# ZECTBynmo/iris-tts

Measured on AMD Instinct MI355X. Metric: audio samples/sec (22.05 kHz) on 80-mel x 1000-frame batch, higher is better.
Workload: dtype f32

## Files before the change

iris-tts_amd/csrc/mrf_pair_bf16.h:

```cpp
#pragma once
#include <stdio.h>
#include "conv_mfma_bf16.h"
#ifndef IRIS_B16_RES_EARLY
#define IRIS_B16_RES_EARLY 1
#endif

#ifndef IRIS_B16_RING_TAIL_GUARD
#define IRIS_B16_RING_TAIL_GUARD 1
#endif
#ifndef IRIS_B16_PAIR_SUM_DEFAULT
#define IRIS_B16_PAIR_SUM_DEFAULT 1
#endif
#ifndef IRIS_B16_SUM32_MT
#define IRIS_B16_SUM32_MT 3
#endif
#ifndef IRIS_B16_SUM64_MT
#define IRIS_B16_SUM64_MT 3
#endif
#ifndef IRIS_B16_SUM32_MINB
#define IRIS_B16_SUM32_MINB 2
#endif
#ifndef IRIS_B16_SUM64_MINB
#define IRIS_B16_SUM64_MINB 2
#endif

namespace iris {
namespace b16 {

struct PairProblem {
    const uint16_t* x;
    const void* w1;
    const void* w2;
    const float* b1;
    const float* b2;
    uint16_t* y;
    int ks;
    int dil;
};

struct PairLaunch {
    PairProblem p[kMaxGroup];
    int B, L, C;
    float slope;
    int nz;
    int Qp, n_ct;
    int n_jobs;
    int jobs_per_xcd;
    int bias_off;
    void* sum_y;
    int sum_f32;
    float inv_n;
};

constexpr int kPairSpanMax = 50;

__device__ __forceinline__ float lrelu_max(float v, float slope) { return fmaxf(v, v * slope); }

template <int NT, int CIC, int D>
__device__ __forceinline__ void ring_request(u32x4 (&wv)[D][NT], __amdgpu_buffer_rsrc_t wr, unsigned wvoff,
                                             unsigned q_bytes, unsigned tap_bytes) {
    constexpr int QPC = CIC / 16;
    constexpr int QL = QPC == 8 ? 3 : (QPC == 4 ? 2 : (QPC == 2 ? 1 : 0));
#pragma unroll
    for (int i = 0; i < D; ++i) {
#pragma unroll
        for (int nt = 0; nt < NT; ++nt)
            wv[i][nt] = buf_load4(wr, wvoff + (unsigned)nt * 1024u, (unsigned)(i >> QL) * tap_bytes + (unsigned)(i & (QPC - 1)) * q_bytes);
        __builtin_amdgcn_sched_barrier(0);
    }
}

template <int MT, int NT, int CIC, int D>
__device__ __forceinline__ void ring_mma_loop(f32x16 (&acc)[MT][NT], u32x4 (&wv)[D][NT], const char* a_lane, int dil_bytes,
                                              __amdgpu_buffer_rsrc_t wr, unsigned wvoff, unsigned q_bytes,
                                              unsigned tap_bytes, int ks) {
    constexpr int QPC = CIC / 16;
    constexpr int QL = QPC == 8 ? 3 : (QPC == 4 ? 2 : (QPC == 2 ? 1 : 0));
    constexpr int SB = CIC * 2 + 16;
    const int NG = ks * QPC;
    auto w_soff = [&](int n) -> unsigned { return (unsigned)(n >> QL) * tap_bytes + (unsigned)(n & (QPC - 1)) * q_bytes; };
    auto load_a = [&](u32x4 (&av)[MT], int n) {
        int tap = n >> QL;
        tap = tap < ks ? tap : ks - 1;
        const char* ap = a_lane + tap * dil_bytes + (n & (QPC - 1)) * 32;
#pragma unroll
        for (int m = 0; m < MT; ++m) av[m] = *reinterpret_cast<const u32x4*>(ap + m * 32 * SB);
    };
    u32x4 av[2][MT];
    load_a(av[0], 0);
    auto group = [&](int i, int n) {
        load_a(av[(i + 1) & 1], n + 1);
        __builtin_amdgcn_sched_barrier(0);
#pragma unroll
        for (int nt = 0; nt < NT; ++nt)
#pragma unroll
            for (int m = 0; m < MT; ++m)
                acc[m][nt] = __builtin_amdgcn_mfma_f32_32x32x16_bf16(
                    __builtin_bit_cast(bf16x8, wv[i][nt]), __builtin_bit_cast(bf16x8, av[i & 1][m]), acc[m][nt], 0, 0, 0);
        __builtin_amdgcn_sched_barrier(0);
#pragma unroll
        for (int nt = 0; nt < NT; ++nt)
            wv[i][nt] = buf_load4(wr, wvoff + (unsigned)nt * 1024u, w_soff(n + D));
    };
    constexpr bool kTail = IRIS_B16_RING_TAIL_GUARD && (QPC % D) != 0;
    const int NG_main = kTail ? (NG / D) * D : NG;
    int n0 = 0;
    for (; n0 < NG_main; n0 += D) {
#pragma unroll
        for (int i = 0; i < D; ++i) group(i, n0 + i);
    }
    if constexpr (kTail) {
        if (n0 < NG) {
#pragma unroll
            for (int i = 0; i < QPC; ++i) group(i, n0 + i);
        }
    }
}

template <int WT, int WC, int MT, int NT, int C, int MINB>
__global__ void __launch_bounds__(256, MINB) mrf_pair_bf16_kernel(const PairLaunch a) {
    extern __shared__ __attribute__((aligned(16))) char lds_pair[];
    char* lds = lds_pair;
    static_assert(WT * WC == 4 && WC * NT * 32 == C, "a block owns all C channels");
    constexpr int SB = C * 2 + 16;
    constexpr int M = WT * MT * 32;
    constexpr int PPR = C / 8;
    constexpr int NQ = ((M + kPairSpanMax) * PPR + 255) / 256;
    constexpr int D = 4;
    const int lane = threadIdx.x & 63, wave = threadIdx.x >> 6;
    const int wt = wave / WC, wc = wave - wt * WC;
    const int lo = lane & 31, hi = lane >> 5;

    const int xcd = blockIdx.x & 7, slot = blockIdx.x >> 3;
    const int job = xcd * a.jobs_per_xcd + slot;
    if (job >= a.n_jobs) return;
    const int tile = job / a.nz, zr = job - tile * a.nz;
    const int z = a.nz - 1 - zr;
    PairProblem p = a.p[0];
    if (z == 1) p = a.p[1];
    if (z == 2) p = a.p[2];
    if (z == 3) p = a.p[3];
    const int ks = p.ks, dil = p.dil;
    const int h2 = (ks - 1) / 2, h1 = dil * (ks - 1) / 2;
    const int T_OUT = M - (ks - 1);
    const int o0 = tile * T_OUT;
    const int L = a.L;
    if (o0 >= L) return;
    const int b = blockIdx.y;
    const int ct0 = wc * NT;

    const unsigned tensor_bytes = (unsigned)L * (unsigned)C * 2u;
    const size_t item = (size_t)b * L * C;
    const unsigned q_bytes = (unsigned)a.n_ct * 1024u;
    const unsigned tap_bytes = (unsigned)a.Qp * q_bytes;
    const unsigned wvoff = (unsigned)ct0 * 1024u + (unsigned)lane * 16u;
    const char* a_lane = lds + (wt * MT * 32 + lo) * SB + hi * 16;
    const __amdgpu_buffer_rsrc_t xr = make_rsrc(p.x + item, tensor_bytes);
    const __amdgpu_buffer_rsrc_t wr1 = make_rsrc(p.w1, (unsigned)ks * tap_bytes);
    const __amdgpu_buffer_rsrc_t wr2 = make_rsrc(p.w2, (unsigned)ks * tap_bytes);

    f32x16 acc[MT][NT];
    auto load_bias = [&](f32x4 (&bias4)[NT][4], const float* bptr) {
#pragma unroll
        for (int nt = 0; nt < NT; ++nt)
#pragma unroll
            for (int g = 0; g < 4; ++g) bias4[nt][g] = *reinterpret_cast<const f32x4*>(bptr + (ct0 + nt) * 32 + 8 * g + 4 * hi);
    };
    auto init_acc = [&](const f32x4 (&bias4)[NT][4]) {
#pragma unroll
        for (int m = 0; m < MT; ++m)
#pragma unroll
            for (int nt = 0; nt < NT; ++nt)
#pragma unroll
                for (int r = 0; r < 16; ++r) acc[m][nt][r] = bias4[nt][r >> 2][r & 3];
    };

    constexpr int RS = NT * 32 * 4 + 16;
    constexpr int PPRO = NT * 4;
    constexpr int NP = 2 * NT;
    const __amdgpu_buffer_rsrc_t yr = make_rsrc(p.y + item, tensor_bytes);
    const __amdgpu_buffer_rsrc_t rr = make_rsrc(p.x + item, tensor_bytes);
    unsigned pvoff[MT][NP];
    int pscr[NP];
    auto geometry = [&](int lane_) {
#pragma unroll
        for (int j = 0; j < NP; ++j) {
            const int q = j * 64 + lane_;
            const int row_l = q / PPRO, pc = q - row_l * PPRO;
            pscr[j] = row_l * RS + pc * 32;
            const int co = ct0 * 32 + 8 * pc;
#pragma unroll
            for (int m = 0; m < MT; ++m) {
                const int im = (wt * MT + m) * 32 + row_l;
                const int o = o0 + im;
                pvoff[m][j] = (im < T_OUT && o < L) ? (unsigned)(o * C + co) * 2u : kOob;
            }
        }
    };
    constexpr int RBUF = IRIS_B16_RES_EARLY ? MT : 2;
    u32x4 resv[RBUF][NP];
    if constexpr (IRIS_B16_RES_EARLY) geometry(lane);
    f32x4 bias4[NT][4];
    load_bias(bias4, p.b1);
    u32x4 wv[D][NT];
    ring_request<NT, C, D>(wv, wr1, wvoff, q_bytes, tap_bytes);
    {
        const int in_row0 = o0 - h2 - h1, R = M + (ks - 1) * dil, total = R * PPR;
        u32x4 v[NQ];
#pragma unroll
        for (int u = 0; u < NQ; ++u) {
            const int idx = u * 256 + (int)threadIdx.x;
            const int r = idx / PPR, pc = idx & (PPR - 1);
            const int row = in_row0 + r;
            const bool ok = idx < total && row >= 0 && row < L;
            v[u] = buf_load4(xr, ok ? (unsigned)(row * C + 8 * pc) * 2u : kOob, 0);
        }
#pragma unroll
        for (int u = 0; u < NQ; ++u) {
            const int idx = u * 256 + (int)threadIdx.x;
            const int r = idx / PPR, pc = idx & (PPR - 1);
            u32x4 o;
#pragma unroll
            for (int e = 0; e < 4; ++e) {
                const unsigned w = v[u][e];
                o[e] = pack_bf2(lrelu_max(bf_lo(w), a.slope), lrelu_max(bf_hi(w), a.slope));
            }
            if (idx < total) *reinterpret_cast<u32x4*>(lds + r * SB + pc * 16) = o;
        }
    }
    if constexpr (IRIS_B16_RES_EARLY) {
#pragma unroll
        for (int m = 0; m < MT; ++m)
#pragma unroll
            for (int j = 0; j < NP; ++j) resv[m][j] = buf_load4(rr, pvoff[m][j], 0);
    }
    __syncthreads();
    init_acc(bias4);
    ring_mma_loop<MT, NT, C, D>(acc, wv, a_lane, dil * SB, wr1, wvoff, q_bytes, tap_bytes, ks);
    ring_request<NT, C, D>(wv, wr2, wvoff, q_bytes, tap_bytes);
    load_bias(bias4, p.b2);
    __syncthreads();
#pragma unroll
    for (int m = 0; m < MT; ++m) {
        const int row_l = (wt * MT + m) * 32 + lo;
        const int row_g = o0 - h2 + row_l;
        const unsigned keep = (row_g >= 0 && row_g < L) ? 0xffffffffu : 0u;
#pragma unroll
        for (int nt = 0; nt < NT; ++nt)
#pragma unroll
            for (int g = 0; g < 4; ++g) {
                u32x2 o;
#pragma unroll
                for (int e2 = 0; e2 < 2; ++e2) {
                    const unsigned t = pack_bf2(acc[m][nt][4 * g + 2 * e2], acc[m][nt][4 * g + 2 * e2 + 1]);
                    o[e2] = pack_bf2(lrelu_max(bf_lo(t), a.slope), lrelu_max(bf_hi(t), a.slope)) & keep;
                }
                *reinterpret_cast<u32x2*>(lds + row_l * SB + ((ct0 + nt) * 32 + 8 * g + 4 * hi) * 2) = o;
            }
    }
    {
        int lane2 = lane;
        if constexpr (IRIS_B16_RES_EARLY) asm volatile("" : "+v"(lane2));
        geometry(lane2);
    }
    if constexpr (!IRIS_B16_RES_EARLY) {
#pragma unroll
        for (int j = 0; j < NP; ++j) resv[0][j] = buf_load4(rr, pvoff[0][j], 0);
    }
    __syncthreads();
    init_acc(bias4);
    ring_mma_loop<MT, NT, C, D>(acc, wv, a_lane, SB, wr2, wvoff, q_bytes, tap_bytes, ks);
    __syncthreads();
    char* scr = lds + wave * (32 * RS);
#pragma unroll
    for (int m = 0; m < MT; ++m) {
        if (!IRIS_B16_RES_EARLY && m + 1 < MT) {
#pragma unroll
            for (int j = 0; j < NP; ++j) resv[(m + 1) & 1][j] = buf_load4(rr, pvoff[m + 1][j], 0);
        }
#pragma unroll
        for (int nt = 0; nt < NT; ++nt)
#pragma unroll
            for (int g = 0; g < 4; ++g) {
                f32x4 v;
#pragma unroll
                for (int e = 0; e < 4; ++e) v[e] = acc[m][nt][4 * g + e];
                *reinterpret_cast<f32x4*>(scr + lo * RS + (nt * 32 + 8 * g + 4 * hi) * 4) = v;
            }
        __builtin_amdgcn_fence(__ATOMIC_RELEASE, "wavefront");
        __builtin_amdgcn_wave_barrier();
        __builtin_amdgcn_fence(__ATOMIC_ACQUIRE, "wavefront");
        u32x4 outp[NP];
#pragma unroll
        for (int j = 0; j < NP; ++j) {
            const f32x4 lo4 = *reinterpret_cast<const f32x4*>(scr + pscr[j]);
            const f32x4 hi4 = *reinterpret_cast<const f32x4*>(scr + pscr[j] + 16);
            const u32x4 rv = resv[IRIS_B16_RES_EARLY ? m : (m & 1)][j];
            outp[j][0] = pack_bf2(lo4[0] + bf_lo(rv[0]), lo4[1] + bf_hi(rv[0]));
            outp[j][1] = pack_bf2(lo4[2] + bf_lo(rv[1]), lo4[3] + bf_hi(rv[1]));
            outp[j][2] = pack_bf2(hi4[0] + bf_lo(rv[2]), hi4[1] + bf_hi(rv[2]));
            outp[j][3] = pack_bf2(hi4[2] + bf_lo(rv[3]), hi4[3] + bf_hi(rv[3]));
        }
        __builtin_amdgcn_sched_barrier(0);
#pragma unroll
        for (int j = 0; j < NP; ++j)
            __builtin_amdgcn_raw_buffer_store_b128(outp[j], yr, (int)pvoff[m][j], 0, 0);
        asm volatile("s_nop 1");
        __builtin_amdgcn_sched_barrier(0);
#pragma unroll
        for (int j = 0; j < NP; ++j) asm volatile("" :: "v"(outp[j]));
        __builtin_amdgcn_fence(__ATOMIC_RELEASE, "wavefront");
        __builtin_amdgcn_wave_barrier();
    }
}

template <int WT, int WC, int MT, int NT, int C, int MINB>
__global__ void __launch_bounds__(256, MINB) mrf_pair_bf16_sum_kernel(const PairLaunch a) {
    extern __shared__ __attribute__((aligned(16))) char lds_pair[];
    char* lds = lds_pair;
    static_assert(WT * WC == 4 && WC * NT * 32 == C, "a block owns all C channels");
    constexpr int SB = C * 2 + 16;
    constexpr int M = WT * MT * 32;
    constexpr int PPR = C / 8;
    constexpr int NQ = ((M + kPairSpanMax) * PPR + 255) / 256;
    constexpr int D = 4;
    constexpr int NZ = 3;
    const int lane = threadIdx.x & 63, wave = threadIdx.x >> 6;
    const int wt = wave / WC, wc = wave - wt * WC;
    const int lo = lane & 31, hi = lane >> 5;
    const int xcd = blockIdx.x & 7, slot = blockIdx.x >> 3;
    const int tile = xcd * a.jobs_per_xcd + slot;
    if (tile >= a.n_jobs) return;
    int kmax = a.p[0].ks;
    if (a.p[1].ks > kmax) kmax = a.p[1].ks;
    if (a.p[2].ks > kmax) kmax = a.p[2].ks;
    const int T_OUT = M - (kmax - 1);
    const int o0 = tile * T_OUT;
    const int L = a.L;
    if (o0 >= L) return;
    const int b = blockIdx.y;
    const int ct0 = wc * NT;
    const unsigned tensor_bytes = (unsigned)L * (unsigned)C * 2u;
    const size_t item = (size_t)b * L * C;
    const unsigned q_bytes = (unsigned)a.n_ct * 1024u;
    const unsigned tap_bytes = (unsigned)a.Qp * q_bytes;
    const unsigned wvoff = (unsigned)ct0 * 1024u + (unsigned)lane * 16u;
    const char* a_lane = lds + (wt * MT * 32 + lo) * SB + hi * 16;

    constexpr int RS = NT * 32 * 4 + 16;
    constexpr int PPRO = NT * 4;
    constexpr int NP = 2 * NT;
    unsigned pvoff[MT][NP];
    int pscr[NP];
#pragma unroll
    for (int j = 0; j < NP; ++j) {
        const int q = j * 64 + lane;
        const int row_l = q / PPRO, pc = q - row_l * PPRO;
        pscr[j] = row_l * RS + pc * 32;
        const int co = ct0 * 32 + 8 * pc;
#pragma unroll
        for (int m = 0; m < MT; ++m) {
            const int im = (wt * MT + m) * 32 + row_l;
            const int o = o0 + im;
            pvoff[m][j] = (im < T_OUT && o < L) ? (unsigned)(o * C + co) * 2u : kOob;
        }
    }
    float sum[MT][NP][8];
    f32x16 acc[MT][NT];
    auto load_bias = [&](f32x4 (&bias4)[NT][4], const float* bptr) {
#pragma unroll
        for (int nt = 0; nt < NT; ++nt)
#pragma unroll
            for (int g = 0; g < 4; ++g) bias4[nt][g] = *reinterpret_cast<const f32x4*>(bptr + (ct0 + nt) * 32 + 8 * g + 4 * hi);
    };
    auto init_acc = [&](const f32x4 (&bias4)[NT][4]) {
#pragma unroll
        for (int m = 0; m < MT; ++m)
#pragma unroll
            for (int nt = 0; nt < NT; ++nt)
#pragma unroll
                for (int r = 0; r < 16; ++r) acc[m][nt][r] = bias4[nt][r >> 2][r & 3];
    };
    char* scr = lds + wave * (32 * RS);

#pragma unroll
    for (int z = 0; z < NZ; ++z) {
        asm volatile("; bf16 summing pair, branch %0" :: "n"(z) : "memory");
        const PairProblem& p = a.p[z];
        const int ks = p.ks, dil = p.dil;
        const int h2 = (ks - 1) / 2, h1 = dil * (ks - 1) / 2;
        const __amdgpu_buffer_rsrc_t xr = make_rsrc(p.x + item, tensor_bytes);
        const __amdgpu_buffer_rsrc_t wr1 = make_rsrc(p.w1, (unsigned)ks * tap_bytes);
        const __amdgpu_buffer_rsrc_t wr2 = make_rsrc(p.w2, (unsigned)ks * tap_bytes);
        if (z > 0) __syncthreads();
        f32x4 bias4[NT][4];
        load_bias(bias4, p.b1);
        u32x4 wv[D][NT];
        ring_request<NT, C, D>(wv, wr1, wvoff, q_bytes, tap_bytes);
        {
            const int in_row0 = o0 - h2 - h1, R = M + (ks - 1) * dil, total = R * PPR;
            u32x4 v[NQ];
#pragma unroll
            for (int u = 0; u < NQ; ++u) {
                const int idx = u * 256 + (int)threadIdx.x;
                const int r = idx / PPR, pc = idx & (PPR - 1);
                const int row = in_row0 + r;
                const bool ok = idx < total && row >= 0 && row < L;
                v[u] = buf_load4(xr, ok ? (unsigned)(row * C + 8 * pc) * 2u : kOob, 0);
            }
#pragma unroll
            for (int u = 0; u < NQ; ++u) {
                const int idx = u * 256 + (int)threadIdx.x;
                const int r = idx / PPR, pc = idx & (PPR - 1);
                u32x4 o;
#pragma unroll
                for (int e = 0; e < 4; ++e) {
                    const unsigned w = v[u][e];
                    o[e] = pack_bf2(lrelu_max(bf_lo(w), a.slope), lrelu_max(bf_hi(w), a.slope));
                }
                if (idx < total) *reinterpret_cast<u32x4*>(lds + r * SB + pc * 16) = o;
            }
        }
        __syncthreads();
        init_acc(bias4);
        ring_mma_loop<MT, NT, C, D>(acc, wv, a_lane, dil * SB, wr1, wvoff, q_bytes, tap_bytes, ks);
        ring_request<NT, C, D>(wv, wr2, wvoff, q_bytes, tap_bytes);
        load_bias(bias4, p.b2);
        __syncthreads();
#pragma unroll
        for (int m = 0; m < MT; ++m) {
            const int row_l = (wt * MT + m) * 32 + lo;
            const int row_g = o0 - h2 + row_l;
            const unsigned keep = (row_g >= 0 && row_g < L) ? 0xffffffffu : 0u;
#pragma unroll
            for (int nt = 0; nt < NT; ++nt)
#pragma unroll
                for (int g = 0; g < 4; ++g) {
                    u32x2 o;
#pragma unroll
                    for (int e2 = 0; e2 < 2; ++e2) {
                        const unsigned t = pack_bf2(acc[m][nt][4 * g + 2 * e2], acc[m][nt][4 * g + 2 * e2 + 1]);
                        o[e2] = pack_bf2(lrelu_max(bf_lo(t), a.slope), lrelu_max(bf_hi(t), a.slope)) & keep;
                    }
                    *reinterpret_cast<u32x2*>(lds + row_l * SB + ((ct0 + nt) * 32 + 8 * g + 4 * hi) * 2) = o;
                }
        }
        const __amdgpu_buffer_rsrc_t rr = make_rsrc(p.x + item, tensor_bytes);
        constexpr int RB = (MT * NT > 3) ? 1 : 2;
        u32x4 resv[RB][NP];
        if (RB == 2) {
#pragma unroll
            for (int j = 0; j < NP; ++j) resv[0][j] = buf_load4(rr, pvoff[0][j], 0);
        }
        __syncthreads();
        init_acc(bias4);
        ring_mma_loop<MT, NT, C, D>(acc, wv, a_lane, SB, wr2, wvoff, q_bytes, tap_bytes, ks);
        __syncthreads();
#pragma unroll
        for (int m = 0; m < MT; ++m) {
            if (RB == 2) {
                if (m + 1 < MT) {
#pragma unroll
                    for (int j = 0; j < NP; ++j) resv[(m + 1) % RB][j] = buf_load4(rr, pvoff[m + 1][j], 0);
                }
            } else {
#pragma unroll
                for (int j = 0; j < NP; ++j) resv[0][j] = buf_load4(rr, pvoff[m][j], 0);
            }
#pragma unroll
            for (int nt = 0; nt < NT; ++nt)
#pragma unroll
                for (int g = 0; g < 4; ++g) {
                    f32x4 v;
#pragma unroll
                    for (int e = 0; e < 4; ++e) v[e] = acc[m][nt][4 * g + e];
                    *reinterpret_cast<f32x4*>(scr + lo * RS + (nt * 32 + 8 * g + 4 * hi) * 4) = v;
                }
            __builtin_amdgcn_fence(__ATOMIC_RELEASE, "wavefront");
            __builtin_amdgcn_wave_barrier();
            __builtin_amdgcn_fence(__ATOMIC_ACQUIRE, "wavefront");
#pragma unroll
            for (int j = 0; j < NP; ++j) {
                const f32x4 lo4 = *reinterpret_cast<const f32x4*>(scr + pscr[j]);
                const f32x4 hi4 = *reinterpret_cast<const f32x4*>(scr + pscr[j] + 16);
                const u32x4 rv = resv[m % RB][j];
                unsigned yp[4];
                yp[0] = pack_bf2(lo4[0] + bf_lo(rv[0]), lo4[1] + bf_hi(rv[0]));
                yp[1] = pack_bf2(lo4[2] + bf_lo(rv[1]), lo4[3] + bf_hi(rv[1]));
                yp[2] = pack_bf2(hi4[0] + bf_lo(rv[2]), hi4[1] + bf_hi(rv[2]));
                yp[3] = pack_bf2(hi4[2] + bf_lo(rv[3]), hi4[3] + bf_hi(rv[3]));
#pragma unroll
                for (int e = 0; e < 4; ++e) {
                    if (z == 0) { sum[m][j][2 * e] = bf_lo(yp[e]); sum[m][j][2 * e + 1] = bf_hi(yp[e]); }
                    else        { sum[m][j][2 * e] = sum[m][j][2 * e] + bf_lo(yp[e]); sum[m][j][2 * e + 1] = sum[m][j][2 * e + 1] + bf_hi(yp[e]); }
                }
            }
            __builtin_amdgcn_fence(__ATOMIC_RELEASE, "wavefront");
            __builtin_amdgcn_wave_barrier();
        }
    }
    if (a.sum_f32) {
        const __amdgpu_buffer_rsrc_t yr = make_rsrc((float*)a.sum_y + item, tensor_bytes * 2u);
#pragma unroll
        for (int m = 0; m < MT; ++m)
#pragma unroll
            for (int j = 0; j < NP; ++j) {
                u32x4 o0v, o1v;
#pragma unroll
                for (int e = 0; e < 4; ++e) {
                    o0v[e] = __builtin_bit_cast(unsigned, (sum[m][j][e] + 0.f) * a.inv_n);
                    o1v[e] = __builtin_bit_cast(unsigned, (sum[m][j][4 + e] + 0.f) * a.inv_n);
                }
                const unsigned vo = pvoff[m][j] == kOob ? kOob : pvoff[m][j] * 2u;
                __builtin_amdgcn_raw_buffer_store_b128(o0v, yr, (int)vo, 0, 0);
                __builtin_amdgcn_raw_buffer_store_b128(o1v, yr, (int)vo, 16, 0);
            }
    } else {
        const __amdgpu_buffer_rsrc_t yr = make_rsrc((uint16_t*)a.sum_y + item, tensor_bytes);
#pragma unroll
        for (int m = 0; m < MT; ++m)
#pragma unroll
            for (int j = 0; j < NP; ++j) {
                u32x4 o;
#pragma unroll
                for (int e = 0; e < 4; ++e)
                    o[e] = pack_bf2(lrelu1((sum[m][j][2 * e] + 0.f) * a.inv_n, a.slope), lrelu1((sum[m][j][2 * e + 1] + 0.f) * a.inv_n, a.slope));
                __builtin_amdgcn_raw_buffer_store_b128(o, yr, (int)pvoff[m][j], 0, 0);
            }
    }
}

struct PairTile { int WT, WC, MT, NT, MINB, M; };

inline bool pair_tile_for(int C, PairTile* t) {
    if (C == 32) {
        *t = PairTile{4, 1, 3, 1, 4, 384};
        return true;
    }
    if (C == 64) {
        *t = PairTile{2, 2, 4, 1, 3, 256};
        return true;
    }
    if (C == 128) { *t = PairTile{2, 2, 3, 2, 2, 192}; return true; }
    return false;
}

inline bool pair_applicable(const PairLaunch& a, int nz) {
    PairTile t;
    if (nz < 1 || nz > kMaxGroup || !pair_tile_for(a.C, &t)) return false;
    if (!(a.slope >= 0.f && a.slope <= 1.f)) return false;
    if ((double)a.L * a.C * 2.0 >= 2147483648.0) return false;
    for (int j = 0; j < nz; ++j) {
        const int ks = a.p[j].ks, d = a.p[j].dil;
        if (ks < 1 || !(ks & 1) || d < 1) return false;
        if (ks - 1 >= t.M / 2) return false;
        if ((ks - 1) * d > kPairSpanMax) return false;
        if ((size_t)(t.M + (ks - 1) * d) * (a.C * 2 + 16) > 66 * 1024) return false;
    }
    return true;
}

inline hipError_t launch_pair_bf16(PairLaunch& a, int nz, hipStream_t stream) {
    PairTile t;
    if (!pair_tile_for(a.C, &t)) return hipErrorInvalidValue;
    for (int j = 0; j < nz; ++j)
        for (int i = 0; i < nz; ++i)
            if (a.p[j].x == a.p[i].y) return hipErrorInvalidValue;
    a.nz = nz;
    a.Qp = packed_qsteps(a.C);
    a.n_ct = packed_cotiles(a.C);
    int span = 0, kmax = 1;
    for (int j = 0; j < nz; ++j) {
        const int s = (a.p[j].ks - 1) * a.p[j].dil;
        if (s > span) span = s;
        if (a.p[j].ks > kmax) kmax = a.p[j].ks;
    }
    const int t_out_min = t.M - (kmax - 1);
    const long long tiles = (a.L + t_out_min - 1) / t_out_min;
    const long long n_jobs = tiles * nz;
    if (n_jobs > 0x3fffffffLL || a.B > 65535) return hipErrorInvalidValue;
    a.n_jobs = (int)n_jobs;
    a.jobs_per_xcd = (int)((n_jobs + 7) / 8);
    const size_t window_bytes = (size_t)(t.M + span) * (a.C * 2 + 16);
    const size_t scratch_bytes = (size_t)4 * 32 * (t.NT * 32 * 4 + 16);
    const size_t lds_bytes = window_bytes > scratch_bytes ? window_bytes : scratch_bytes;
    dim3 grid((unsigned)(a.jobs_per_xcd * 8), (unsigned)a.B, 1u), block(256);
#define IRIS_PAIR_CASE(WT_, WC_, MT_, NT_, C_, MINB_)                                                        \
    if (a.C == C_ && t.WT == WT_ && t.WC == WC_ && t.MT == MT_ && t.NT == NT_ && t.MINB == MINB_) {        \
        auto kfn = mrf_pair_bf16_kernel<WT_, WC_, MT_, NT_, C_, MINB_>;                                      \
        { const hipError_t e__ = ::iris::launch_kernel_named("mrf_pair_bf16_kernel", kfn, grid, block, lds_bytes, stream, a); if (e__ != hipSuccess) return e__; } \
        return hipSuccess;                                                                                   \
    }
    IRIS_PAIR_CASE(4, 1, 3, 1, 32, 4)
    IRIS_PAIR_CASE(2, 2, 4, 1, 64, 3)
    IRIS_PAIR_CASE(2, 2, 3, 2, 128, 2)
#undef IRIS_PAIR_CASE
    return hipErrorInvalidValue;
}

inline bool pair_sum_tile_for(int C, PairTile* t) {
    if (C == 32)  { *t = PairTile{4, 1, IRIS_B16_SUM32_MT, 1, IRIS_B16_SUM32_MINB, 4 * IRIS_B16_SUM32_MT * 32}; return true; }
    if (C == 64)  { *t = PairTile{2, 2, IRIS_B16_SUM64_MT, 1, IRIS_B16_SUM64_MINB, 2 * IRIS_B16_SUM64_MT * 32}; return true; }
    return false;
}

inline bool pair_sum_applicable(const PairLaunch& a, int nz, bool f32_out) {
    PairTile t;
    if (nz != 3 || !pair_sum_tile_for(a.C, &t)) return false;
    if (!(a.slope >= 0.f && a.slope <= 1.f)) return false;
    if ((double)a.L * a.C * (f32_out ? 4.0 : 2.0) >= 2147483648.0) return false;
    for (int j = 0; j < nz; ++j) {
        const int ks = a.p[j].ks, d = a.p[j].dil;
        if (ks < 1 || !(ks & 1) || d < 1) return false;
        if (ks - 1 >= t.M / 2) return false;
        if ((ks - 1) * d > kPairSpanMax) return false;
        if ((size_t)(t.M + (ks - 1) * d) * (a.C * 2 + 16) > 66 * 1024) return false;
    }
    return IRIS_B16_PAIR_SUM_DEFAULT != 0;
}

inline hipError_t launch_pair_bf16_sum(PairLaunch& a, void* sum_y, bool f32_out, hipStream_t stream) {
    PairTile t;
    if (!pair_sum_tile_for(a.C, &t) || !sum_y) return hipErrorInvalidValue;
    for (int j = 0; j < 3; ++j)
        if ((const void*)a.p[j].x == sum_y) return hipErrorInvalidValue;
    a.nz = 3;
    a.Qp = packed_qsteps(a.C);
    a.n_ct = packed_cotiles(a.C);
    a.sum_y = sum_y; a.sum_f32 = f32_out ? 1 : 0; a.inv_n = 1.0f / 3.0f;
    int span = 0, kmax = 1;
    for (int j = 0; j < 3; ++j) {
        const int s = (a.p[j].ks - 1) * a.p[j].dil;
        if (s > span) span = s;
        if (a.p[j].ks > kmax) kmax = a.p[j].ks;
    }
    const int t_out = t.M - (kmax - 1);
    const long long tiles = (a.L + t_out - 1) / t_out;
    if (tiles > 0x3fffffffLL || a.B > 65535) return hipErrorInvalidValue;
    a.n_jobs = (int)tiles;
    a.jobs_per_xcd = (int)((tiles + 7) / 8);
    const size_t window_bytes = (size_t)(t.M + span) * (a.C * 2 + 16);
    const size_t scratch_bytes = (size_t)4 * 32 * (t.NT * 32 * 4 + 16);
    const size_t lds_bytes = window_bytes > scratch_bytes ? window_bytes : scratch_bytes;
    dim3 grid((unsigned)(a.jobs_per_xcd * 8), (unsigned)a.B, 1u), block(256);
#define IRIS_PAIR_SUM_CASE(WT_, WC_, MT_, NT_, C_, MINB_)                                                    \
    if (a.C == C_ && t.WT == WT_ && t.WC == WC_ && t.MT == MT_ && t.NT == NT_ && t.MINB == MINB_) {        \
        auto kfn = mrf_pair_bf16_sum_kernel<WT_, WC_, MT_, NT_, C_, MINB_>;                                  \
        { const hipError_t e__ = ::iris::launch_kernel_named("mrf_pair_bf16_sum_kernel", kfn, grid, block, lds_bytes, stream, a); if (e__ != hipSuccess) return e__; } \
        return hipSuccess;                                                                                   \
    }
    IRIS_PAIR_SUM_CASE(4, 1, IRIS_B16_SUM32_MT, 1, 32, IRIS_B16_SUM32_MINB)
    IRIS_PAIR_SUM_CASE(2, 2, IRIS_B16_SUM64_MT, 1, 64, IRIS_B16_SUM64_MINB)
#undef IRIS_PAIR_SUM_CASE
    return hipErrorInvalidValue;
}

}
}
```

Before: 53.37 million.

## Prefetch next branch's input window and all residual rows during conv2 MMA

Moves the global loads of the next branch's input window and first weight ring out of the branch prologue. They are now issued right after the second conv's MMA loop, so they overlap the epilogue and summation. All residual rows are also loaded up front, into a buffer sized MT, instead of one or two at a time. This hides load latency across branch boundaries but raises VGPR pressure (v[NQ], resv[MT][NP], and the live wv). The added asm barriers pin the sum registers and the scheduling order, and the extra registers may lower occupancy or cause spills.

New measurement: 53.33 million (median of 2 runs). Within noise of the previous version (-0.1%).

```diff
diff --git a/iris-tts_amd/csrc/mrf_pair_bf16.h b/iris-tts_amd/csrc/mrf_pair_bf16.h
--- a/iris-tts_amd/csrc/mrf_pair_bf16.h
+++ b/iris-tts_amd/csrc/mrf_pair_bf16.h
@@ -22,6 +22,9 @@
 #endif
 #ifndef IRIS_B16_SUM64_MINB
 #define IRIS_B16_SUM64_MINB 2
+#endif
+#ifndef IRIS_B16_SUM_WINDOW_EARLY
+#define IRIS_B16_SUM_WINDOW_EARLY 1
 #endif
 
 namespace iris {
@@ -383,44 +386,54 @@
     };
     char* scr = lds + wave * (32 * RS);
 
+    constexpr bool kEarly = IRIS_B16_SUM_WINDOW_EARLY != 0;
+    u32x4 wv[D][NT];
+    u32x4 v[NQ];
+    auto window_request = [&](const PairProblem& p) {
+        const int ks = p.ks, dil = p.dil;
+        const int h2 = (ks - 1) / 2, h1 = dil * (ks - 1) / 2;
+        const __amdgpu_buffer_rsrc_t xr = make_rsrc(p.x + item, tensor_bytes);
+        const __amdgpu_buffer_rsrc_t wr1 = make_rsrc(p.w1, (unsigned)ks * tap_bytes);
+        ring_request<NT, C, D>(wv, wr1, wvoff, q_bytes, tap_bytes);
+        const int in_row0 = o0 - h2 - h1, R = M + (ks - 1) * dil, total = R * PPR;
+#pragma unroll
+        for (int u = 0; u < NQ; ++u) {
+            const int idx = u * 256 + (int)threadIdx.x;
+            const int r = idx / PPR, pc = idx & (PPR - 1);
+            const int row = in_row0 + r;
+            const bool ok = idx < total && row >= 0 && row < L;
+            v[u] = buf_load4(xr, ok ? (unsigned)(row * C + 8 * pc) * 2u : kOob, 0);
+        }
+    };
+    auto window_write = [&](const PairProblem& p) {
+        const int total = (M + (p.ks - 1) * p.dil) * PPR;
+#pragma unroll
+        for (int u = 0; u < NQ; ++u) {
+            const int idx = u * 256 + (int)threadIdx.x;
+            const int r = idx / PPR, pc = idx & (PPR - 1);
+            u32x4 o;
+#pragma unroll
+            for (int e = 0; e < 4; ++e) {
+                const unsigned w = v[u][e];
+                o[e] = pack_bf2(lrelu_max(bf_lo(w), a.slope), lrelu_max(bf_hi(w), a.slope));
+            }
+            if (idx < total) *reinterpret_cast<u32x4*>(lds + r * SB + pc * 16) = o;
+        }
+    };
+
 #pragma unroll
     for (int z = 0; z < NZ; ++z) {
         asm volatile("; bf16 summing pair, branch %0" :: "n"(z) : "memory");
         const PairProblem& p = a.p[z];
         const int ks = p.ks, dil = p.dil;
-        const int h2 = (ks - 1) / 2, h1 = dil * (ks - 1) / 2;
-        const __amdgpu_buffer_rsrc_t xr = make_rsrc(p.x + item, tensor_bytes);
+        const int h2 = (ks - 1) / 2;
         const __amdgpu_buffer_rsrc_t wr1 = make_rsrc(p.w1, (unsigned)ks * tap_bytes);
         const __amdgpu_buffer_rsrc_t wr2 = make_rsrc(p.w2, (unsigned)ks * tap_bytes);
         if (z > 0) __syncthreads();
         f32x4 bias4[NT][4];
         load_bias(bias4, p.b1);
-        u32x4 wv[D][NT];
-        ring_request<NT, C, D>(wv, wr1, wvoff, q_bytes, tap_bytes);
-        {
-            const int in_row0 = o0 - h2 - h1, R = M + (ks - 1) * dil, total = R * PPR;
-            u32x4 v[NQ];
-#pragma unroll
-            for (int u = 0; u < NQ; ++u) {
-                const int idx = u * 256 + (int)threadIdx.x;
-                const int r = idx / PPR, pc = idx & (PPR - 1);
-                const int row = in_row0 + r;
-                const bool ok = idx < total && row >= 0 && row < L;
-                v[u] = buf_load4(xr, ok ? (unsigned)(row * C + 8 * pc) * 2u : kOob, 0);
-            }
-#pragma unroll
-            for (int u = 0; u < NQ; ++u) {
-                const int idx = u * 256 + (int)threadIdx.x;
-                const int r = idx / PPR, pc = idx & (PPR - 1);
-                u32x4 o;
-#pragma unroll
-                for (int e = 0; e < 4; ++e) {
-                    const unsigned w = v[u][e];
-                    o[e] = pack_bf2(lrelu_max(bf_lo(w), a.slope), lrelu_max(bf_hi(w), a.slope));
-                }
-                if (idx < total) *reinterpret_cast<u32x4*>(lds + r * SB + pc * 16) = o;
-            }
-        }
+        if (!kEarly || z == 0) window_request(p);
+        window_write(p);
         __syncthreads();
         init_acc(bias4);
         ring_mma_loop<MT, NT, C, D>(acc, wv, a_lane, dil * SB, wr1, wvoff, q_bytes, tap_bytes, ks);
@@ -446,19 +459,29 @@
                 }
         }
         const __amdgpu_buffer_rsrc_t rr = make_rsrc(p.x + item, tensor_bytes);
-        constexpr int RB = (MT * NT > 3) ? 1 : 2;
+        constexpr int RB = kEarly ? MT : ((MT * NT > 3) ? 1 : 2);
         u32x4 resv[RB][NP];
-        if (RB == 2) {
+        if (kEarly || RB == 2) {
 #pragma unroll
             for (int j = 0; j < NP; ++j) resv[0][j] = buf_load4(rr, pvoff[0][j], 0);
         }
         __syncthreads();
         init_acc(bias4);
         ring_mma_loop<MT, NT, C, D>(acc, wv, a_lane, SB, wr2, wvoff, q_bytes, tap_bytes, ks);
+        if constexpr (kEarly) {
+#pragma unroll
+            for (int m = 1; m < MT; ++m)
+#pragma unroll
+                for (int j = 0; j < NP; ++j) resv[m][j] = buf_load4(rr, pvoff[m][j], 0);
+            __builtin_amdgcn_sched_barrier(0);
+            if (z + 1 < NZ) window_request(a.p[z + 1]);
+            __builtin_amdgcn_sched_barrier(0);
+        }
         __syncthreads();
 #pragma unroll
         for (int m = 0; m < MT; ++m) {
-            if (RB == 2) {
+            if constexpr (kEarly) {
+            } else if (RB == 2) {
                 if (m + 1 < MT) {
 #pragma unroll
                     for (int j = 0; j < NP; ++j) resv[(m + 1) % RB][j] = buf_load4(rr, pvoff[m + 1][j], 0);
@@ -493,6 +516,10 @@
                 for (int e = 0; e < 4; ++e) {
                     if (z == 0) { sum[m][j][2 * e] = bf_lo(yp[e]); sum[m][j][2 * e + 1] = bf_hi(yp[e]); }
                     else        { sum[m][j][2 * e] = sum[m][j][2 * e] + bf_lo(yp[e]); sum[m][j][2 * e + 1] = sum[m][j][2 * e + 1] + bf_hi(yp[e]); }
+                }
+                if constexpr (kEarly) {
+#pragma unroll
+                    for (int e = 0; e < 8; ++e) asm volatile("" : "+v"(sum[m][j][e]));
                 }
             }
             __builtin_amdgcn_fence(__ATOMIC_RELEASE, "wavefront");
```
